# IntelLabs/GKL

Hardware: AMD Instinct MI355X
Metric: pairhmm_gcups (higher is better)
Workload: dtype f32

## Files before the change

gkl_amd/csrc/pairhmm_aux_kernels.h:

```cpp
#pragma once
#include <hip/hip_runtime.h>
#include <stdint.h>

#include "../../include/gkl_hip_pairhmm.h"
#include "pairhmm_fwd_kernel.h"
#include "pairhmm_multi_sets.h"

namespace gklhip {

struct PrepArgs {
  const uint8_t* hap_bases;
  const int32_t* hap_src;
  const int32_t* hap_len;
  const int32_t* hap_pos;
  const int32_t* hap_group;
  const int32_t* hap_pos_flat;
  uint32_t* stream_flat;
  uint32_t* stream;
  uint8_t* hap_has_n;
  int32_t n_haps;
  int32_t* clear_a; int32_t n_a;
  int32_t* clear_b; int32_t n_b;
  int32_t* clear_c; int32_t n_c;
  const uint4* pull_src; uint4* pull_dst; int32_t pull_n16;
// ... 166 lines not shown
  a.b.del = global_ptr(a.b.del); a.b.gcp = global_ptr(a.b.gcp); a.b.read_off = global_ptr(a.b.read_off);
  a.tab.ph2pr = global_ptr(a.tab.ph2pr); a.tab.div3 = global_ptr(a.tab.div3); a.tab.mm = global_ptr(a.tab.mm);
  a.stream = global_ptr(a.stream); a.hap_len = global_ptr(a.hap_len); a.hap_pos = global_ptr(a.hap_pos);
  a.hap_orig = global_ptr(a.hap_orig); a.y0 = global_ptr(a.y0); a.hap_has_n = global_ptr(a.hap_has_n);
  a.groups = global_ptr(a.groups); a.chunk_lanes = global_ptr(a.chunk_lanes); a.raw = global_ptr(a.raw);
  fwd_stream_block<double, kRplJobs, FMA>(a, block, lds);
}
__global__ __launch_bounds__(kFlagBlock) void finalize64_multi_kernel(MultiArgs m) {
  const int r = multi_find(m, (int)blockIdx.x);
  const SmallCall* c = m.call[r];
  const int p = multi_local(m.begin, r, (int)blockIdx.x) * kFlagBlock + (int)threadIdx.x;
  if (p >= c->n_pairs) return;
  c->q.used64[p] = 1;
  reinterpret_cast<uint64_t*>(c->q.out)[p] = packed_word(c->d.raw[p]);
}

constexpr int kModePacked = kModePackedWords;

struct FinalizeArgs {
  const float* raw32;
  const double* raw64;
  double* out;
  uint8_t* used64;
  int32_t* count;
  int32_t* read_fail;
  int32_t n_haps;
  int64_t n;
  int mode;
  float log10_init_f;
  double log10_init32_as_f64;
  double log10_init_d;
};

__global__ void finalize32_kernel(FinalizeArgs a) {
  const int64_t i = (int64_t)blockIdx.x * blockDim.x + threadIdx.x;
  if (i >= a.n || a.used64[i]) return;
  const float v = a.raw32[i];
  if (a.mode == GKLHIP_FINALIZE_DEVICE_F64) a.out[i] = log10((double)v) - a.log10_init32_as_f64;
  else if (a.mode == GKLHIP_FINALIZE_DEVICE_REF32) a.out[i] = (double)((float)log10((double)v) - a.log10_init_f);
}

__global__ void finalize64_kernel(FinalizeArgs a, int all_pairs) {
  const int64_t p = (int64_t)blockIdx.x * blockDim.x + threadIdx.x;
  if (p >= a.n) return;
  if (all_pairs) a.used64[p] = 1;
  else if (!a.used64[p]) return;
  if (a.mode >= 0) a.out[p] = log10(a.raw64[p]) - a.log10_init_d;
  if (a.mode == kModePacked) reinterpret_cast<uint64_t*>(a.out)[p] = packed_word(a.raw64[p]);
}

#ifndef GKL_PACK_WINDOW
#define GKL_PACK_WINDOW 96
#endif
constexpr int kPackWindow = GKL_PACK_WINDOW;
constexpr int kJobClasses = 64;
constexpr int kPlanBlock = 1024;

struct PlanArgs {
  FinalizeArgs fa;
  int32_t n_reads, n_haps, n_pairs_i;
  const int64_t* read_off;
  int32_t rpl;
  int32_t max_len;
  int32_t* cnts;
  int32_t* hist;
  int32_t* pos;
  int32_t* order;
  LaneSlot* lanes2;
  const int32_t* hap_orig;
  const int32_t* hap_group;
  const int32_t* hap_pos;
  const int32_t* hap_len;
  FwdJob* jobs;
  FwdJob* sorted;
  const LaneSlot* long_lanes;
  int32_t n_long;
  FwdJob* jobs_long;
  int32_t* long_chunk_jobs;
  int32_t total_cols;
  int32_t wanted_jobs;
  int32_t min_job_cols;
// ... 142 lines not shown
    for (int k = 0; k < kBatch; k++)
      if (f[k] > 0) a.order[atomicAdd(pos + f[k], 1)] = r0 + k * kPlanBlock;
  }
}

__global__ __launch_bounds__(kPlanBlock) void plan_policy_kernel(PlanArgs a) {
  __shared__ int32_t s_i32[kPlanBlock / 64];
  __shared__ int32_t s_wave[kPlanBlock / 64];
  __shared__ int32_t s_hist[2 * kPlanLdsBins];
  const int tid = (int)threadIdx.x, lane = tid & 63, wave = tid >> 6;
  const int nblk = (int)gridDim.x, blk = (int)blockIdx.x;

  {
    int32_t my_fails = 0;
    for (int64_t base = (int64_t)blk * kPlanBlock; base < a.fa.n; base += (int64_t)nblk * kPlanBlock) {
      const int64_t i = base + tid;
      const bool in_range = i < a.fa.n;
      const float v = in_range ? a.fa.raw32[i] : 1.0f;
      const bool fails = in_range && v < 1e-28f;
      const uint64_t mask = __ballot(fails);
      if (mask) {
        const int leader = __builtin_ctzll(mask);
        const int32_t read = fails ? (int32_t)((uint32_t)i / (uint32_t)a.n_haps) : -1;
        const int32_t lead_read = __shfl(read, leader, 64);
        const uint64_t same = __ballot(fails && read == lead_read);
        if (lane == leader) atomicAdd(a.fa.read_fail + lead_read, __builtin_popcountll(same));
        if (fails && read != lead_read) atomicAdd(a.fa.read_fail + read, 1);
        if (lane == 0) my_fails += __builtin_popcountll(mask);
      }
      if (in_range) {
        a.fa.used64[i] = fails ? 1 : 0;
        if (a.fa.mode == kModePacked && !a.packed_by_kernels)
          reinterpret_cast<uint64_t*>(a.fa.out)[i] = fails ? 0ull : (kPackedF32Tag | (uint64_t)__float_as_uint(v));
      }
    }
    if (lane == 0) s_wave[wave] = my_fails;
    __syncthreads();
    if (tid == 0) {
      int total = 0;
      for (int w = 0; w < kPlanBlock / 64; w++) total += s_wave[w];
      if (total) atomicAdd(a.cnts + 0, total);
    }
  }
  if (!last_block_done(a.cnts + 10)) return;
  const int n_fail = ld_cnt(a.cnts + 0);
  if (n_fail == 0) return;
  const uint64_t clk0 = wall_clock64();

  if (a.n_haps + 2 <= kPlanLdsBins) order_affected_reads<true>(a, s_hist, s_hist + kPlanLdsBins, s_i32, tid, clk0);
  else                             order_affected_reads<false>(a, a.hist, a.pos, s_i32, tid, clk0);
  GKLHIP_PLAN_STAMP(2);
}

__global__ __launch_bounds__(kPlanBlock) void plan_pack_kernel(PlanArgs a) {
  const int tid = (int)threadIdx.x, lane = tid & 63, wave = tid >> 6;
  const int nblk = (int)gridDim.x, blk = (int)blockIdx.x;
  if (ld_cnt(a.cnts + 0) == 0) return;
  const uint64_t clk0 = wall_clock64();

  {
    static_assert(kPackWindow <= 2 * kLanes, "the window's lane counts sit in two registers per lane");
    __shared__ int32_t s_pack[kPlanBlock / 64][4][kPackWindow];
    int32_t* s_read = s_pack[wave][0]; int32_t* s_needl = s_pack[wave][1]; int32_t* s_sread = s_pack[wave][2];
    int32_t* s_sneed = s_pack[wave][3];
    const int n = ld_cnt(a.cnts + 4);
    const int n_win = (n + kPackWindow - 1) / kPackWindow;
// ... 360 lines not shown
```

gkl_amd/csrc/pairhmm_ctx.h:

```cpp
#pragma once

using namespace gklhip;

namespace {
struct EnvSwitches {
  static bool on_unless_zero(const char* name) { const char* v = getenv(name); return !v || atoi(v) != 0; }
  static int integer(const char* name) { const char* v = getenv(name); return v ? atoi(v) : 0; }
  const bool wide_long = on_unless_zero("GKLHIP_WIDE_LONG");
  const bool super_long = on_unless_zero("GKLHIP_SUPER_LONG");
  const bool fused_pairs = on_unless_zero("GKLHIP_FUSED_PAIRS");
  const int64_t fused_max = [] { const char* v = getenv("GKLHIP_FUSED_MAX_PAIRS"); return v ? atoll(v) : -1LL; }();
  const bool xcd_aware = on_unless_zero("GKLHIP_XCD_AWARE");
  const bool timing = getenv("GKLHIP_TIMING") != nullptr;
  const int combine_load = integer("GKL_HIP_COMBINE_LOAD");
  const int target_cols = integer("GKLHIP_TARGET_COLS");
  const int fb_wanted_jobs = integer("GKLHIP_FB_WANTED_JOBS");
  const int plan_blocks = integer("GKLHIP_PLAN_BLOCKS");
  const int finalize_threads = integer("GKL_HIP_FINALIZE_THREADS");
  const int finalize_min = integer("GKL_HIP_FINALIZE_MIN");
  const bool combine = [] { const char* v = getenv("GKL_HIP_COMBINE"); return !(v && v[0] == '0'); }();
  const bool combine_mid = integer("GKL_HIP_COMBINE_MID") != 0;
  const bool quiet = getenv("GKL_HIP_QUIET") != nullptr;
  const bool one_device_engine = integer("GKL_HIP_DEVICE_ENGINES") == 1;
  const int small_read_limit = integer("GKL_HIP_SMALL_READ_LIMIT") == 511 ? 511 : 383;
// ... 3 lines not shown

#include "hip_host_common.h"

struct DevCtx {
  gklhip_config cfg;
  int device = 0;
  bool multi_device = false;
  int n_cus = 256;
  int n_xcds = 8;
  int asm_general = 1;
  int speculate_fp64 = 0;
  int small_read_limit = g_env.small_read_limit;
  int mid_combine = g_env.combine_mid ? 1 : 0;
  int lds_oob_zero = 1;
  hipStream_t stream = nullptr;
  DevBuf tab32, tab64;
  DevTables<float> dt32;
  DevTables<double> dt64;
  PinBuf stage_slot[2];
  DevBuf plan_dev_slot[2];
  hipEvent_t stage_free_slot[2] = {nullptr, nullptr};
  hipEvent_t plan_unused_slot[2] = {nullptr, nullptr};
  hipStream_t upload_stream = nullptr;
  bool upload_eager = false;
  hipStream_t pad_stream = nullptr;
  int plan_slot = 0;
  DevBuf raw32, raw64, used64, counters, stream_buf, out_dev;
  DevBuf lanes_main;
  DevBuf read_fail, lanes2, jobs, jobs_long, fail_order, fail_hist, hap_flags;
  DevBuf batch_dev;
  PinBuf res_pin;
  WorkerPool workers;
  hipStream_t copy_stream = nullptr;
  hipEvent_t policy_done = nullptr, early_copy_done = nullptr;
  hipEvent_t call_done = nullptr;
  bool have_call_done = false;
  static constexpr int kEventRing = 64;
  hipEvent_t ev_ring[kEventRing][6] = {};
  hipEvent_t* ev = ev_ring[0];
  int64_t calls = 0;
  bool ring_double[kEventRing] = {};
  gklhip_stats stats;
  int64_t last_pairs = 0;
  hipStream_t last_stream = nullptr;
  bool have_last = false;
  Plan plan;
  std::vector<PlanLane> long_lanes;
  std::vector<FwdJob> long_jobs;
  DevBuf carry;
};
```

gkl_amd/csrc/pairhmm_ctx_lifecycle.h:

```cpp
#pragma once

namespace {

std::atomic<int> g_eager_upload_holders{0};

int trim_streams(DevCtx* c) {
  if (!c->copy_stream && !c->pad_stream && (!c->upload_stream || c->upload_eager)) return 0;
  (void)hipSetDevice(c->device);
  for (hipStream_t s : {c->stream, c->copy_stream, c->upload_stream, c->have_last ? c->last_stream : nullptr})
    if (s && hipStreamQuery(s) != hipSuccess) { (void)hipGetLastError(); return 0; }
  int n = 0;
  if (c->copy_stream) { (void)hipStreamDestroy(c->copy_stream); c->copy_stream = nullptr; n++; }
  if (c->pad_stream) { (void)hipStreamDestroy(c->pad_stream); c->pad_stream = nullptr; n++; }
  if (c->upload_stream && !c->upload_eager) { (void)hipStreamDestroy(c->upload_stream); c->upload_stream = nullptr; n++; }
  return n;
}

void dev_done(DevCtx* c) {
  if (!c) return;
  (void)hipSetDevice(c->device);
  if (c->upload_eager) g_eager_upload_holders--;
  if (c->stream) (void)hipStreamSynchronize(c->stream);
  if (c->last_stream && c->have_last) (void)hipStreamSynchronize(c->last_stream);
  for (DevBuf* b : {&c->tab32, &c->tab64, &c->plan_dev_slot[0], &c->plan_dev_slot[1], &c->raw32, &c->raw64, &c->used64,
                    &c->counters, &c->stream_buf, &c->out_dev, &c->batch_dev, &c->read_fail, &c->lanes_main,
                    &c->lanes2, &c->jobs, &c->jobs_long, &c->fail_order, &c->fail_hist, &c->carry, &c->hap_flags})
    b->release();
  c->stage_slot[0].release();
  c->stage_slot[1].release();
  c->res_pin.release();
  if (c->policy_done) (void)hipEventDestroy(c->policy_done);
  if (c->early_copy_done) (void)hipEventDestroy(c->early_copy_done);
  if (c->call_done) (void)hipEventDestroy(c->call_done);
  if (c->copy_stream) { (void)hipStreamSynchronize(c->copy_stream); (void)hipStreamDestroy(c->copy_stream); }
  for (auto& set : c->ev_ring)
    for (auto& e : set) if (e) (void)hipEventDestroy(e);
  for (int k = 0; k < 2; k++) {
    if (c->stage_free_slot[k]) (void)hipEventDestroy(c->stage_free_slot[k]);
    if (c->plan_unused_slot[k]) (void)hipEventDestroy(c->plan_unused_slot[k]);
  }
  if (c->upload_stream) { (void)hipStreamSynchronize(c->upload_stream); (void)hipStreamDestroy(c->upload_stream); }
  if (c->pad_stream) (void)hipStreamDestroy(c->pad_stream);
  if (c->stream) (void)hipStreamDestroy(c->stream);
  delete c;
}

int dev_init(const gklhip_config& cfg, int dev, int ndev, DevCtx** out) {
  *out = nullptr;
  if (dev < 0 || dev >= ndev) return fail(GKLHIP_ERR_INVALID_ARG, "device %d of %d", dev, ndev);
  HIP_TRY(hipSetDevice(dev));
  {
    static const char* sched = getenv("GKL_HIP_SCHEDULE");
    if (sched && *sched) {
      const unsigned f = strcmp(sched, "yield") == 0 ? hipDeviceScheduleYield : strcmp(sched, "blocking") == 0 ? hipDeviceScheduleBlockingSync
                         : strcmp(sched, "spin") == 0 ? hipDeviceScheduleSpin : hipDeviceScheduleAuto;
      (void)hipSetDeviceFlags(f);
      (void)hipGetLastError();
    }
  }
  hipDeviceProp_t prop;
  HIP_TRY(hipGetDeviceProperties(&prop, dev));
  if (strncmp(prop.gcnArchName, "gfx950", 6) != 0)
    return fail(GKLHIP_ERR_NO_DEVICE, "device %d is %s; this library is built for gfx950 only", dev, prop.gcnArchName);
  DevCtx* c = new (std::nothrow) DevCtx();
  if (!c) return fail(GKLHIP_ERR_OOM, "context allocation failed");
  c->cfg = cfg;
// ... 35 lines not shown
      if (oob_checked[(size_t)dev] < 0)
        fprintf(stderr, "[gklhip] pairhmm: LDS reads beyond the allocation do not return 0 on device %d (%08x): the fp32 general steps stay in C++\n", dev, h_out[2]);
    }
    if (checked[(size_t)dev] < 0)
      return bail(fail(GKLHIP_ERR_HIP, "this library was built without the denormal-flush flags its kernels depend on (gkl_amd/csrc/Makefile: HIPFLAGS)"));
    c->lds_oob_zero = oob_checked[(size_t)dev] > 0 ? 1 : 0;
  }
  {
    const char* ag = getenv("GKLHIP_ASM_GENERAL");
    c->asm_general = ag ? (atoi(ag) != 0) : 1;
    const char* sp = getenv("GKLHIP_SPECULATE_FP64");
    c->speculate_fp64 = sp ? (atoi(sp) != 0) : 0;
    const char* sf = getenv("GKLHIP_SELFTEST_FAIL");
    if (sf && strcmp(sf, "lds_oob") == 0) {
      c->lds_oob_zero = 0;
      fprintf(stderr, "[gklhip] pairhmm: GKLHIP_SELFTEST_FAIL=lds_oob: the fp32 general steps stay in C++ for this context\n");
    }
  }
  if (g_eager_upload_holders.fetch_add(1) == 0) {
    if (hipStreamCreateWithFlags(&c->upload_stream, hipStreamNonBlocking) != hipSuccess) { g_eager_upload_holders--; return bail(fail(GKLHIP_ERR_HIP, "hipStreamCreate failed")); }
    c->upload_eager = true;
  } else {
    g_eager_upload_holders--;
  }
  if (const char* v = getenv("GKL_HIP_EAGER_STREAMS")) {
    const int k = atoi(v);
    if (k >= 7) { if (aux_streams(c) != GKLHIP_OK) return bail(GKLHIP_ERR_HIP); }
    else for (int i = 0; i < k; i++) { hipStream_t d = nullptr; (void)hipStreamCreateWithFlags(&d, hipStreamNonBlocking); }
  }
  for (int k = 0; k < 2; k++)
    if (hipEventCreateWithFlags(&c->stage_free_slot[k], hipEventDisableTiming) != hipSuccess ||
        hipEventCreateWithFlags(&c->plan_unused_slot[k], hipEventDisableTiming) != hipSuccess)
      return bail(fail(GKLHIP_ERR_HIP, "hipEventCreate failed"));
  if (hipEventCreateWithFlags(&c->policy_done, hipEventDisableTiming) != hipSuccess ||
      hipEventCreateWithFlags(&c->early_copy_done, hipEventDisableTiming) != hipSuccess ||
      hipEventCreateWithFlags(&c->call_done, hipEventDisableTiming) != hipSuccess)
    return bail(fail(GKLHIP_ERR_HIP, "hipEventCreate failed"));
  for (int k = 0; k < 2; k++)
    if (hipEventRecord(c->stage_free_slot[k], c->stream) != hipSuccess || hipEventRecord(c->plan_unused_slot[k], c->stream) != hipSuccess)
      return bail(fail(GKLHIP_ERR_HIP, "hipEventRecord failed"));
  {
    const int sets = c->cfg.record_events == 2 ? DevCtx::kEventRing : 1;
    for (int k = 0; k < sets; k++)
      for (auto& e : c->ev_ring[k])
        if (hipEventCreate(&e) != hipSuccess) return bail(fail(GKLHIP_ERR_HIP, "hipEventCreate failed"));
  }
  if ((rc = upload_tables(c, host_tables_f32(), &c->tab32, &c->dt32))) return bail(rc);
  if ((rc = upload_tables(c, host_tables_f64(), &c->tab64, &c->dt64))) return bail(rc);
  *out = c;
  return GKLHIP_OK;
}

int lane_init(DevCtx* parent, DevCtx** out) {
  *out = nullptr;
  HIP_TRY(hipSetDevice(parent->device));
  DevCtx* c = new (std::nothrow) DevCtx();
  if (!c) return fail(GKLHIP_ERR_OOM, "context allocation failed");
  c->cfg = parent->cfg;
  c->device = parent->device;
  c->n_cus = parent->n_cus;
  c->n_xcds = parent->n_xcds;
  c->asm_general = parent->asm_general;
  c->speculate_fp64 = parent->speculate_fp64;
  c->small_read_limit = parent->small_read_limit;
  c->mid_combine = parent->mid_combine;
  c->lds_oob_zero = parent->lds_oob_zero;
  c->dt32 = parent->dt32;
  c->dt64 = parent->dt64;
  memset(&c->stats, 0, sizeof c->stats);
// ... 14 lines not shown
```

gkl_amd/csrc/pairhmm_device_pass.h:

```cpp
#pragma once

namespace {

int aux_streams(DevCtx* c) {
  if (!c->upload_stream) HIP_TRY(hipStreamCreateWithFlags(&c->upload_stream, hipStreamNonBlocking));
  if (!c->copy_stream) {
    HIP_TRY(hipStreamCreateWithFlags(&c->copy_stream, hipStreamNonBlocking));
    if (!c->pad_stream) HIP_TRY(hipStreamCreateWithFlags(&c->pad_stream, hipStreamNonBlocking));
  }
  return GKLHIP_OK;
}

template <typename T>
int upload_tables(DevCtx* c, const HostTables<T>& h, DevBuf* buf, DevTables<T>* dt) {
  const size_t n = (size_t)kQuals * 2 + kMmEntries;
  int st = buf->reserve(n * sizeof(T));
  if (st) return st;
  T* base = buf->as<T>();
  {
    T* pin = nullptr;
    HIP_TRY(hipHostMalloc(reinterpret_cast<void**>(&pin), n * sizeof(T), hipHostMallocDefault));
    memcpy(pin, h.ph2pr.data(), kQuals * sizeof(T));
    memcpy(pin + kQuals, h.div3.data(), kQuals * sizeof(T));
    memcpy(pin + 2 * kQuals, h.mm.data(), kMmEntries * sizeof(T));
// ... 51 lines not shown
  l.desc = o; if (inline_read_bytes) o = align_up(o + sizeof(SmallCall));
  l.total = o;
  return l;
}

int validate(const gklhip_batch* b) {
  if (!b) return fail(GKLHIP_ERR_INVALID_ARG, "batch is NULL");
  if (b->n_reads < 0 || b->n_haps < 0) return fail(GKLHIP_ERR_INVALID_ARG, "negative batch size");
  if (b->n_reads == 0 || b->n_haps == 0) return GKLHIP_OK;
  if (!b->read_off || !b->hap_off) return fail(GKLHIP_ERR_INVALID_ARG, "offset arrays are NULL");
  if (!b->read_bases || !b->read_quals || !b->ins_gop || !b->del_gop || !b->gcp || !b->hap_bases)
    return fail(GKLHIP_ERR_INVALID_ARG, "a batch byte array is NULL");
  if (b->read_off[0] != 0 || b->hap_off[0] != 0)
    return fail(GKLHIP_ERR_INVALID_ARG, "offset arrays must start at 0");
  for (int r = 0; r < b->n_reads; r++)
    if (b->read_off[r + 1] <= b->read_off[r])
      return fail(GKLHIP_ERR_INVALID_ARG, "read %d is empty or offsets are not increasing", r);
  for (int h = 0; h < b->n_haps; h++)
    if (b->hap_off[h + 1] <= b->hap_off[h])
      return fail(GKLHIP_ERR_INVALID_ARG, "haplotype %d is empty or offsets are not increasing", h);
  if ((int64_t)b->n_reads * b->n_haps >= (int64_t)1 << 31)
    return fail(GKLHIP_ERR_UNSUPPORTED, "more than 2^31 pairs in one call");
  if (b->hap_off[b->n_haps] + b->n_haps + 4096 >= (int64_t)1 << 31)
    return fail(GKLHIP_ERR_UNSUPPORTED, "haplotype bases exceed 2^31");
  return GKLHIP_OK;
}

template <typename T, int RPL>
void launch_stream(const FwdArgs<T>& a, int fma, int n_blocks, hipStream_t s) {
  if (fma) hipLaunchKernelGGL((pairhmm_fwd_stream_kernel<T, RPL, true>), dim3(n_blocks), dim3(64), 0, s, a);
  else     hipLaunchKernelGGL((pairhmm_fwd_stream_kernel<T, RPL, false>), dim3(n_blocks), dim3(64), 0, s, a);
}
template <typename T, int RPL>
void launch_jobs(const FwdArgs<T>& a, int fma, int n_blocks, hipStream_t s) {
  if (fma) hipLaunchKernelGGL((pairhmm_fwd_jobs_kernel<T, RPL, true>), dim3(n_blocks), dim3(64), 0, s, a);
  else     hipLaunchKernelGGL((pairhmm_fwd_jobs_kernel<T, RPL, false>), dim3(n_blocks), dim3(64), 0, s, a);
}

template <typename T, int RPL>
void launch_long(const FwdArgs<T>& a, int fma, int n_blocks, T* carry, int carry_len, hipStream_t s) {
  if (fma) hipLaunchKernelGGL((pairhmm_fwd_long_kernel<T, RPL, true>), dim3(n_blocks), dim3(64), 0, s, a, carry, carry_len);
  else     hipLaunchKernelGGL((pairhmm_fwd_long_kernel<T, RPL, false>), dim3(n_blocks), dim3(64), 0, s, a, carry, carry_len);
}

template <typename T> constexpr int super_waves() { return 7; }
template <typename T> constexpr int super_blocks_max() { return sizeof(T) == 8 ? 256 : 512; }
inline int64_t super_steps(int carry_len, int max_read_len, int rpl) { return (int64_t)carry_len + 64 * (int64_t)((blocks_for(max_read_len, rpl) + kLanes - 1) / kLanes); }
template <typename T, int RPL, int RPL_STRIPED>
void launch_long_jobs(const FwdArgs<T>& a, int fma, int n_blocks, int max_read_len, T* carry, int carry_len, hipStream_t s,
                      unsigned char* xcarry = nullptr, int64_t xsteps = 0, int32_t* next2 = nullptr) {
  const bool wide_env = g_env.wide_long, super_env = g_env.super_long;
  if (!wide_env) { launch_long<T, RPL_STRIPED>(a, fma, n_blocks, carry, carry_len, s); return; }
  if (super_env && xcarry && next2 && (blocks_for(max_read_len, RPL) + kLanes - 1) / kLanes > kWideWavesMax) {
    static_assert(RPL == kRplSuper, "the super-stripe kernel's array depth");
    FwdArgs<T> sa = a;
    sa.super_steps = xsteps;
    if (fma) hipLaunchKernelGGL((pairhmm_fwd_super_kernel<T, RPL, super_waves<T>(), true>), dim3(std::min(n_blocks, super_blocks_max<T>())), dim3(64 * (super_waves<T>() + 1)), 0, s, sa, xcarry);
    else     hipLaunchKernelGGL((pairhmm_fwd_super_kernel<T, RPL, super_waves<T>(), false>), dim3(std::min(n_blocks, super_blocks_max<T>())), dim3(64 * (super_waves<T>() + 1)), 0, s, sa, xcarry);
    sa.long_filter = 2;
    sa.job_next = next2;
    launch_long<T, RPL_STRIPED>(sa, fma, n_blocks, carry, carry_len, s);
    return;
  }
  const int waves = std::max(2, std::min(kWideWavesMax, (blocks_for(max_read_len, RPL) + kLanes - 1) / kLanes));
  if (fma) {
    if (waves == 2)      hipLaunchKernelGGL((pairhmm_fwd_wide_kernel<T, RPL, true, 2>), dim3(n_blocks), dim3(128), 0, s, a, carry, carry_len);
    else if (waves == 3) hipLaunchKernelGGL((pairhmm_fwd_wide_kernel<T, RPL, true, 3>), dim3(n_blocks), dim3(192), 0, s, a, carry, carry_len);
    else                 hipLaunchKernelGGL((pairhmm_fwd_wide_kernel<T, RPL, true, 4>), dim3(n_blocks), dim3(256), 0, s, a, carry, carry_len);
  } else {
// ... 301 lines not shown
    copy_six_arrays(*db, L.batch_stride, [dst](size_t at, const uint8_t* src, size_t n) { memcpy(dst + at, src, n); return 0; });
    build_host_streams(hs, L, plan, db->hap_bases, n_haps);
  }
}

struct StagedCall {
  hipStream_t s;
  double* out;
  int slot;
  unsigned char* hs;
  const unsigned char* hs_dev;
  unsigned char* dp;
  DevBatch b;
  const uint8_t* hap_bases;
  uint32_t *stream_grouped, *stream_flat;
  uint8_t *hap_has_n, *xcarry;
};

int stage_call(DevCtx* c, const gklhip_batch* db, const CallPlan& P, double* out_dev, hipStream_t s, StagedCall* out) {
  const PlanLayout& L = P.L;
  const Plan& plan = c->plan;
  StagedCall& S = *out;
  int rc;
  const int slot = c->plan_slot ^= 1;
  PinBuf& stage = c->stage_slot[slot];
  DevBuf& plan_dev = c->plan_dev_slot[slot];
  HIP_TRY(hipEventSynchronize(c->stage_free_slot[slot]));
  if (L.total > stage.cap || L.total > plan_dev.cap) HIP_TRY(hipEventSynchronize(c->plan_unused_slot[slot]));
  if ((rc = stage.reserve(L.total))) return rc;
  if ((rc = plan_dev.reserve(L.total))) return rc;
  unsigned char* hs = stage.as<unsigned char>();
  fill_plan_block(hs, P, plan, c->long_lanes, c->long_jobs, db);
  unsigned char* dp = plan_dev.as<unsigned char>();
  if (c->have_call_done && c->last_stream != s) HIP_TRY(hipStreamWaitEvent(s, c->call_done, 0));
  S.hs_dev = nullptr;
  if (P.pull) {
    void* p = nullptr;
    HIP_TRY(hipHostGetDevicePointer(&p, hs, 0));
    S.hs_dev = static_cast<const unsigned char*>(p);
    if (!P.defers) HIP_TRY(hipStreamWaitEvent(s, c->plan_unused_slot[slot], 0));
  } else {
    if ((rc = aux_streams(c))) return rc;
    HIP_TRY(hipStreamWaitEvent(c->upload_stream, c->plan_unused_slot[slot], 0));
    HIP_TRY(hipMemcpyAsync(dp, hs, L.total, hipMemcpyHostToDevice, c->upload_stream));
    HIP_TRY(hipEventRecord(c->stage_free_slot[slot], c->upload_stream));
    HIP_TRY(hipStreamWaitEvent(s, c->stage_free_slot[slot], 0));
  }
  if (g_env.timing)
    fprintf(stderr, "[gklhip] host plan + staging: %.3f ms (%d chunks, %d stream entries, %zu plan bytes)\n",
            std::chrono::duration<double, std::milli>(std::chrono::steady_clock::now() - P.t0).count(),
            plan.n_chunks, plan.n_stream, L.total);

  if ((rc = c->raw32.reserve((size_t)P.n_pairs * 4))) return rc;
  if ((rc = c->raw64.reserve((size_t)P.n_pairs * 8))) return rc;
  if ((rc = c->used64.reserve((size_t)P.n_pairs))) return rc;
  if ((rc = c->counters.reserve(128))) return rc;
  if ((rc = c->read_fail.reserve((size_t)P.n_reads * 4))) return rc;
  if ((rc = c->stream_buf.reserve(((size_t)plan.n_stream + (size_t)plan.n_stream_flat) * 4))) return rc;
  if (!P.use_double && (rc = c->fail_hist.reserve((size_t)P.n_hist * 4))) return rc;
  if ((rc = c->hap_flags.reserve((size_t)P.n_haps))) return rc;
  if ((rc = c->lanes_main.reserve((size_t)std::max(plan.n_chunks, 1) * kLanes * sizeof(LaneSlot)))) return rc;

  S.s = s; S.out = out_dev; S.slot = slot; S.hs = hs; S.dp = dp; S.xcarry = nullptr;
  const gklhip_batch dbi = P.inline_host ? batch_at(*db, dp + L.batch, L.batch_stride) : *db;
  S.b = DevBatch{dbi.read_bases, dbi.read_quals, dbi.ins_gop, dbi.del_gop, dbi.gcp, reinterpret_cast<const int64_t*>(dp + L.read_off), P.n_reads, P.n_haps};
  S.hap_bases = (P.pull && P.inline_host) ? batch_at(*db, S.hs_dev + L.batch, L.batch_stride).hap_bases : dbi.hap_bases;
  S.stream_grouped = P.inline_host ? reinterpret_cast<uint32_t*>(dp + L.stream) : c->stream_buf.as<uint32_t>();
// ... 189 lines not shown
  if (P.fused) {
    if (int rc = launch_pair_fused(a, d, q, P.rows, P.fma, P.n_pairs, s, c->speculate_fp64 && g_host_calls_in_flight.load(std::memory_order_relaxed) <= 1)) return rc;
  } else if (P.n_pairs > kTwoStepFrom) {
    if (int rc = c->fail_order.reserve((size_t)P.n_pairs * 4)) return rc;
    if (int rc = launch_pair_policy_two_step(d, q, P.rows, P.fma, P.n_pairs, c->fail_order.as<int32_t>(), s)) return rc;
  } else {
    if (int rc = launch_pair_policy(d, q, P.rows, P.fma, P.n_pairs, s)) return rc;
  }
  if (ev) HIP_TRY(hipEventRecord(c->ev[4], s));
  HIP_TRY(hipEventRecord(c->policy_done, s));
  return GKLHIP_OK;
}
int launch_planned_fp64(DevCtx* c, const CallPlan& P, const StagedCall& S) {
  const bool ev = c->cfg.record_events != 0;
  hipStream_t s = S.s;
  const int n_reads = P.n_reads;
  const int64_t n_pairs = P.n_pairs;
  const size_t max_jobs = planned_max_jobs(P);
  int rc;
  if ((rc = c->fail_order.reserve(((size_t)n_reads + (size_t)P.n_long64) * 4))) return rc;
  if ((rc = c->lanes2.reserve((size_t)n_reads * kLanes * sizeof(LaneSlot)))) return rc;
  if ((rc = c->jobs.reserve(2 * max_jobs * sizeof(FwdJob)))) return rc;
  if (P.n_long64 > 0 && (rc = c->jobs_long.reserve((size_t)P.n_long64 * (size_t)P.n_haps * sizeof(FwdJob)))) return rc;
  const PlanArgs pa = plan_args(c, P, S);
  const int blocks_env = g_env.plan_blocks;
  const int policy_grid = std::max(1, blocks_env > 0 ? blocks_env : (int)std::min<int64_t>(c->n_cus, std::max<int64_t>(16, n_pairs / 4096)));
  const int64_t max_windows = ((int64_t)n_reads + kPackWindow - 1) / kPackWindow;
  const int pack_grid = (int)std::max<int64_t>(1, std::min<int64_t>(kPlanBlocks, (max_windows + kPlanBlock / 64 - 1) / (kPlanBlock / 64)));
  const int jobs_grid = std::max(1, std::min(c->n_cus, blocks_env > 0 ? blocks_env : (int)std::min<int64_t>(kPlanBlocks, std::max<int64_t>(16, n_pairs / 8192))));
  hipLaunchKernelGGL(plan_policy_kernel, dim3((unsigned)policy_grid), dim3(kPlanBlock), 0, s, pa);
  HIP_TRY(hipEventRecord(c->policy_done, s));
  hipLaunchKernelGGL(plan_pack_kernel, dim3((unsigned)pack_grid), dim3(kPlanBlock), 0, s, pa);
  hipLaunchKernelGGL(plan_jobs_kernel, dim3((unsigned)jobs_grid), dim3(kPlanBlock), 0, s, pa);
  const bool side_finalize = finalizes_on_device(P.finalize_mode);
  if (side_finalize) {
    if ((rc = aux_streams(c))) return rc;
    HIP_TRY(hipStreamWaitEvent(c->copy_stream, c->policy_done, 0));
    hipLaunchKernelGGL(finalize32_kernel, dim3((unsigned)((n_pairs + 255) / 256)), dim3(256), 0, c->copy_stream, pa.fa);
    HIP_TRY(hipEventRecord(c->early_copy_done, c->copy_stream));
  }
  FwdArgs<double> d = recompute_args(c, P, S);
  d.chunk_lanes = c->lanes2.as<LaneSlot>();
  d.n_chunks = n_reads;
  d.jobs = c->jobs.as<FwdJob>() + max_jobs;
  if (ev) HIP_TRY(hipEventRecord(c->ev[3], s));
  launch_jobs<double, kRplF64Jobs>(d, P.fma, (int)std::min<int64_t>(n_pairs, (int64_t)c->n_cus * 16), s);
  if (P.n_long64 > 0) {
    int32_t* cnts = c->counters.as<int32_t>();
    FwdArgs<double> ld = d;
    ld.chunk_lanes = pa.long_lanes;
    ld.jobs = c->jobs_long.as<FwdJob>();
    ld.job_count = cnts + 8;
    ld.job_next = cnts + 9;
    launch_long_jobs<double, kRplF64Wide, kRplF64>(ld, P.fma, P.n_long_waves, c->plan.max_read_len, c->carry.as<double>(), P.carry_len, s, S.xcarry, P.xsteps, cnts + 13);
  }
  if (ev) HIP_TRY(hipEventRecord(c->ev[4], s));
  hipLaunchKernelGGL(finalize64_kernel, dim3((unsigned)((n_pairs + 255) / 256)), dim3(256), 0, s, pa.fa, 0);
  if (side_finalize) HIP_TRY(hipStreamWaitEvent(s, c->early_copy_done, 0));
  return GKLHIP_OK;
}
int finish_call(DevCtx* c, const CallPlan& P, const StagedCall& S) {
  const bool ev = c->cfg.record_events != 0;
  hipStream_t s = S.s;
  gklhip_stats& st = c->stats;
  if (ev) HIP_TRY(hipEventRecord(c->ev[5], s));
  HIP_TRY(hipGetLastError());

  HIP_TRY(hipEventRecord(c->plan_unused_slot[S.slot], s));
  HIP_TRY(hipEventRecord(c->call_done, s));
  c->have_call_done = true;
  c->last_pairs = P.n_pairs;
  c->last_stream = s;
  c->have_last = true;

  if (ev && c->cfg.record_events != 2) {
    HIP_TRY(hipEventSynchronize(c->ev[5]));
    float ms = 0;
    HIP_TRY(hipEventElapsedTime(&ms, c->ev[1], c->ev[2])); st.ms_fwd_main = ms;
    HIP_TRY(hipEventElapsedTime(&ms, c->ev[3], c->ev[4])); st.ms_fwd_fallback = P.use_double ? 0.f : ms;
    HIP_TRY(hipEventElapsedTime(&ms, c->ev[0], c->ev[5])); st.ms_total_device = ms;
    int32_t cnt[2] = {0, 0};
    HIP_TRY(hipMemcpyAsync(cnt, c->counters.p, 8, hipMemcpyDeviceToHost, s));
    HIP_TRY(hipStreamSynchronize(s));
    st.n_fallback = P.use_double ? P.n_pairs : cnt[0];
    if (g_env.timing && !P.use_double) {
      int32_t k[32];
      HIP_TRY(hipMemcpy(k, c->counters.p, sizeof k, hipMemcpyDeviceToHost));
      fprintf(stderr, "[gklhip] policy+plan phases, each from the start of its own launch (us): hist %.1f scan %.1f scatter %.1f pack %.1f jobs %.1f sort %.1f | "
              "%d affected reads, %d chunks, %d jobs | window 0: loaded %.1f ranked %.1f fitted %.1f cleared %.1f written %.1f\n",
              k[16] * 0.01, k[17] * 0.01, k[18] * 0.01, k[19] * 0.01, k[20] * 0.01, k[21] * 0.01,
              k[4], k[5], k[2], k[22] * 0.01, k[23] * 0.01, k[24] * 0.01, k[25] * 0.01, k[26] * 0.01);
    }
  } else {
    st.n_fallback = P.use_double ? P.n_pairs : -1;
  }
  return GKLHIP_OK;
}

int32_t small_call_kind(const CallPlan& P) {
  if (P.use_double && P.n_pairs > kSmallDoublePairs) return kSmallDoubleStream;
  return P.pair_double ? kSmallDouble : P.fused ? kSmallFused : P.n_pairs > kTwoStepFrom ? kSmallTwoStep : kSmallOneLaunch;
}
// ... 53 lines not shown
```

gkl_amd/csrc/pairhmm_fwd_kernel.h:

```cpp
#pragma once
#include <hip/hip_runtime.h>
#include <stdint.h>

#include "pairhmm_pair_forms.h"

namespace gklhip {

constexpr uint32_t kEntIdle = 5u;
constexpr uint32_t kEntSep = 0x80000000u;
constexpr int kLanes = kPairLanes;
typedef const uint32_t __attribute__((address_space(4))) StreamWord;
}
#include "pairhmm_fwd_asm.h"
#ifndef GKLHIP_FAST_ASM
#define GKLHIP_FAST_ASM 1
#endif
namespace gklhip {

template <typename T>
struct DevTables {
  const T* ph2pr;
  const T* div3;
  const T* mm;
};
// ... 22 lines not shown
  int32_t klass;
};

template <typename T>
struct FwdArgs {
  DevBatch b;
  DevTables<T> tab;
  const uint32_t* stream;
  const int32_t* hap_len;
  const int32_t* hap_pos;
  const int32_t* hap_orig;
  const T* y0;
  const uint8_t* hap_has_n;
  const HapGroup* groups;
  int32_t n_groups;
  const LaneSlot* chunk_lanes;
  int32_t n_chunks;
  int32_t chunk_stride;
  T* raw;
  uint64_t* packed_out;
  const uint8_t* packed_only_flagged;
  const FwdJob* jobs;
  const int32_t* job_count;
  int32_t* job_next;
  int32_t asm_general;
  int32_t long_filter;
  int64_t super_steps;
};

constexpr uint64_t kPackedF32Tag = 0xFFFFFFFF00000000ull;
__device__ __forceinline__ uint64_t packed_word(double raw) {
  const uint64_t bits = (uint64_t)__double_as_longlong(raw);
  return (bits & kPackedF32Tag) == kPackedF32Tag ? 0x7FF8000000000000ull : bits;
}

template <typename T>
__device__ __forceinline__ void emit_result(const FwdArgs<T>& a, int64_t idx, T v) {
  a.raw[idx] = v;
  if (a.packed_out) {
    if (sizeof(T) == 4) {
      const float f = (float)v;
      a.packed_out[idx] = f < 1e-28f ? 0ull : (kPackedF32Tag | (uint64_t)__float_as_uint(f));
    } else if (!a.packed_only_flagged || a.packed_only_flagged[idx]) {
      a.packed_out[idx] = packed_word((double)v);
    }
  }
}

__device__ __forceinline__ uint32_t dpp_shr1_keep(uint32_t old, uint32_t src) {
  return (uint32_t)__builtin_amdgcn_update_dpp((int)old, (int)src, 0x138, 0xf, 0xf, false);
}
__device__ __forceinline__ uint32_t dpp_shr1_zero(uint32_t src) {
  return (uint32_t)__builtin_amdgcn_update_dpp(0, (int)src, 0x138, 0xf, 0xf, true);
}
__device__ __forceinline__ uint32_t dpp_shr1_and_nop(uint32_t src, uint32_t mask) {
  uint32_t d;
  asm("s_nop 1\n\tv_and_b32_dpp %0, %1, %2 wave_shr:1 row_mask:0xf bank_mask:0xf bound_ctrl:1" : "=v"(d) : "v"(src), "v"(mask));
  return d;
}
__device__ __forceinline__ float recv_above(float v, uint32_t lmask) {
  return __uint_as_float(dpp_shr1_and_nop(__float_as_uint(v), lmask));
}
__device__ __forceinline__ double recv_above(double v, uint32_t lmask) {
  const uint64_t u = (uint64_t)__double_as_longlong(v);
  const uint32_t lo = dpp_shr1_zero((uint32_t)u) & lmask;
  const uint32_t hi = dpp_shr1_zero((uint32_t)(u >> 32)) & lmask;
// ... 434 lines not shown
          const T bM = read_lane(M[RPL - 1], kLanes - 1), bX = read_lane(X[RPL - 1], kLanes - 1),
                  bY = read_lane(Y[RPL - 1], kLanes - 1);
          if (lane == (p & 63)) { coM = bM; coX = bX; coY = bY; }
          if ((p & 63) == 63 || t == t_end - 1) {
            const int base = p & ~63;
            cout[base + lane] = coM; cout[clen + base + lane] = coX; cout[2 * clen + base + lane] = coY;
          }
        }
      }
    }
  }
};

template <typename T, int RPL, bool FMA>
__device__ __forceinline__ void fwd_stream_block(const FwdArgs<T>& a, int block, unsigned char* lds) {
  using Job = WaveJob<T, RPL, FMA>;
  const int lane = threadIdx.x;
  const int g = block / a.chunk_stride;
  const int chunk = block - g * a.chunk_stride;
  if (chunk >= a.n_chunks) return;
  const HapGroup grp = a.groups[g];
  Job job;
  job.lds = lds;
  job.setup(a, lane, a.chunk_lanes[(int64_t)chunk * kLanes + lane]);
  __syncthreads();
  job.run(a, lane, grp.hap_begin, grp.hap_end);
}
template <typename T, int RPL, bool FMA>
__global__ __launch_bounds__(64) __attribute__((amdgpu_waves_per_eu(sizeof(T) == 8 ? 2 : 4))) void pairhmm_fwd_stream_kernel(FwdArgs<T> a) {
  __shared__ __attribute__((aligned(16))) unsigned char lds[WaveJob<T, RPL, FMA>::kLdsBytes];
  fwd_stream_block<T, RPL, FMA>(a, (int)blockIdx.x, lds);
}

template <typename T, int RPL, bool FMA>
__global__ __launch_bounds__(64) __attribute__((amdgpu_waves_per_eu(sizeof(T) == 8 ? 2 : 4))) void pairhmm_fwd_jobs_kernel(FwdArgs<T> a) {
  using Job = WaveJob<T, RPL, FMA>;
  __shared__ __attribute__((aligned(16))) unsigned char lds[Job::kLdsBytes];
  const int lane = threadIdx.x;
  const int n = *a.job_count;
  Job job;
  job.lds = lds;
  int loaded_chunk = INT32_MIN;
  for (;;) {
    int idx = 0;
    if (lane == 0) idx = atomicAdd(a.job_next, 1);
    idx = __builtin_amdgcn_readfirstlane(idx);
    if (idx >= n) break;
    const FwdJob j = a.jobs[idx];
    if (j.chunk != loaded_chunk) {
      __syncthreads();
      job.setup(a, lane, a.chunk_lanes[(int64_t)j.chunk * kLanes + lane]);
      __syncthreads();
      loaded_chunk = j.chunk;
    }
    job.run(a, lane, j.hap_begin, j.hap_end);
  }
}

struct PairPolicyArgs {
  const float* raw32;
  double* out;
  uint8_t* used64;
  int32_t* count;
  const int32_t* hap_sidx;
  int32_t mode;
  float log10_init_f;
  double log10_init32_as_f64, log10_init_d;
};
constexpr int kModePackedWords = -2;

__device__ __forceinline__ void pair_store_fp32(const PairPolicyArgs& q, int64_t p, float v) {
  if (q.mode == kModePackedWords) reinterpret_cast<uint64_t*>(q.out)[p] = kPackedF32Tag | (uint64_t)__float_as_uint(v);
  else if (q.mode == 1) q.out[p] = log10((double)v) - q.log10_init32_as_f64;
  else if (q.mode == 2) q.out[p] = (double)((float)log10((double)v) - q.log10_init_f);
}
__device__ __forceinline__ bool pair_policy_head(const PairPolicyArgs& q, int64_t p, int lane) {
  const float v = q.raw32[p];
  const bool fails = v < 1e-28f;
  if (lane == 0) q.used64[p] = fails ? 1 : 0;
  if (!fails) {
    if (lane == 0) pair_store_fp32(q, p, v);
    return false;
  }
  if (lane == 0) atomicAdd(q.count, 1);
  return true;
}
template <int RPL, bool FMA, bool MARK = false>
__device__ __forceinline__ void pair_policy_recompute(const FwdArgs<double>& a, const PairPolicyArgs& q, int64_t p, int r, int R, int k,
                                                      unsigned char* lds) {
  using Job = WaveJob<double, RPL, FMA>;
  const int lane = threadIdx.x & 63;
  LaneSlot slot;
  slot.read = lane < (R + RPL) / RPL ? r : -1;
  slot.block = lane;
  Job job;
  job.lds = lds;
  job.setup(a, lane, slot);
  __builtin_amdgcn_wave_barrier();
  job.run(a, lane, k, k + 1);
  if (job.out_read >= 0) {
    const double sum = a.raw[p];
    if (q.mode == kModePackedWords) reinterpret_cast<uint64_t*>(q.out)[p] = packed_word(sum);
// ... 449 lines not shown
```

gkl_amd/csrc/pairhmm_host_call.h:

```cpp
#pragma once

namespace {

struct HostCallInFlight {
  int share;
  HostCallInFlight() : share(g_host_calls_in_flight.fetch_add(1) + 1) {}
  ~HostCallInFlight() { g_host_calls_in_flight.fetch_sub(1); }
};
int finalize_threads(const DevCtx* c, int share) {
  const int env = g_env.finalize_threads;
  if (env > 0) return env;
  const int hw = (int)std::max(1u, std::thread::hardware_concurrency());
  int threads = c->cfg.max_threads;
  if (threads <= 0) threads = std::max(1, std::min(hw, 8) / std::max(1, share));
  return std::max(1, std::min(threads, 64));
}

constexpr int kFlightSlots = 4;
struct SmallCombiner {
  struct Ticket {
    const SmallLaunch* sl = nullptr;
    int state = 0;
    hipEvent_t ev = nullptr;
    int rc = GKLHIP_OK;
// ... 216 lines not shown
    }
    l.unlock();
    if (t.state == 2) { g_err = t.err; return t.rc; }
    if (t.state == 1) HIP_TRY(hipEventSynchronize(t.ev));
    return GKLHIP_OK;
  }
};
SmallCombiner* small_combiner(int device) {
  static std::mutex mu;
  static std::vector<SmallCombiner*> all;
  std::lock_guard<std::mutex> l(mu);
  if ((int)all.size() <= device) all.resize((size_t)device + 1, nullptr);
  if (!all[(size_t)device]) {
    SmallCombiner* k = all[(size_t)device] = new SmallCombiner();
    k->device = device;
    if (const char* v = getenv("GKL_HIP_EAGER_STREAMS")) if (atoi(v) >= 7) k->make_streams();
    if (const char* v = getenv("GKL_HIP_COMBINE_FLIGHTS")) all[(size_t)device]->max_flights = std::max(1, std::min(kFlightSlots, atoi(v)));
    if (const char* v = getenv("GKL_HIP_COMBINE_MIN")) all[(size_t)device]->min_batch = std::max(0, std::min(kCombineMax, atoi(v)));
    if (const char* v = getenv("GKL_HIP_COMBINE_WAIT_US")) all[(size_t)device]->batch_wait_ns = (int64_t)std::max(0, atoi(v)) * 1000;
  }
  return all[(size_t)device];
}
int64_t one_pass_min() { return g_env.finalize_min > 0 ? g_env.finalize_min : 8192; }
int dev_compute_host_impl(DevCtx* c, const gklhip_batch* hb, double* out_host) {
  const int64_t n_pairs = (int64_t)hb->n_reads * hb->n_haps;
  HIP_TRY(hipSetDevice(c->device));
  hipStream_t s = c->stream;
  int rc;
  const bool inline_inputs = inputs_inline(hb);
  gklhip_batch db = *hb;
  if (!inline_inputs) {
    if ((rc = c->batch_dev.reserve(six_arrays_bytes(hb)))) return rc;
    unsigned char* d = c->batch_dev.as<unsigned char>();
    if (c->have_call_done && c->last_stream != s) HIP_TRY(hipStreamWaitEvent(s, c->call_done, 0));
    const size_t stride = align_up((size_t)hb->read_off[hb->n_reads]);
    if ((rc = copy_six_arrays(*hb, stride, [d, s](size_t at, const uint8_t* src, size_t n) -> int { HIP_TRY(hipMemcpyAsync(d + at, src, n, hipMemcpyHostToDevice, s)); return GKLHIP_OK; }))) return rc;
    db = batch_at(*hb, d, stride);
  }
  const int mode = c->cfg.finalize;
  if ((rc = c->res_pin.reserve((size_t)n_pairs * 8))) return rc;
  double* pin_out = nullptr;
  {
    void* p = nullptr;
    HIP_TRY(hipHostGetDevicePointer(&p, c->res_pin.p, 0));
    pin_out = static_cast<double*>(p);
  }
  if (finalizes_on_device(mode)) {
    if ((rc = run_device(c, &db, pin_out, mode, s, inline_inputs))) return rc;
    HIP_TRY(hipStreamSynchronize(s));
    memcpy(out_host, c->res_pin.p, (size_t)n_pairs * 8);
    return GKLHIP_OK;
  }
  const HostCallInFlight in_flight;
  const int threads = finalize_threads(c, in_flight.share);
  HostFinalizer fin;
  const bool may_defer = deferral_offered(inline_inputs) && (!c->have_call_done || hipEventQuery(c->call_done) == hipSuccess);
  (void)hipGetLastError();
  const int64_t t_call = SmallCombiner::now_ns();
  CallPlan P;
  plan_call(c, &db, kModePacked, inline_inputs, may_defer, call_load(may_defer), &P);
  const bool mid = !P.defers && may_defer && mid_call_combines(c, P);
  if (mid) P.defers = true;
  if (P.defers) {
    StagedCall S;
    SmallLaunch small;
    if ((rc = stage_call(c, &db, P, pin_out, s, &S))) return rc;
    if (mid && !P.use_double && (rc = c->fail_order.reserve((size_t)P.n_pairs * 4))) return rc;
    describe_small_call(c, P, S, &small);
    SmallCombiner* k = small_combiner(c->device);
    const int64_t t_staged = SmallCombiner::now_ns();
    if ((rc = k->run(small, s))) return rc;
    const int64_t t_done = SmallCombiner::now_ns();
    c->stats.n_fallback = fin.all(&c->workers, c->res_pin.as<uint64_t>(), out_host, n_pairs, threads, one_pass_min());
    k->ns_stage.fetch_add(t_staged - t_call, std::memory_order_relaxed);
    k->ns_run.fetch_add(t_done - t_staged, std::memory_order_relaxed);
    k->ns_finalize.fetch_add(SmallCombiner::now_ns() - t_done, std::memory_order_relaxed);
    return GKLHIP_OK;
  }
  if ((rc = launch_call(c, &db, P, pin_out, s))) return rc;
  if (c->cfg.use_double || n_pairs <= kOnePassPairs) {
    HIP_TRY(hipStreamSynchronize(s));
    c->stats.n_fallback = fin.all(&c->workers, c->res_pin.as<uint64_t>(), out_host, n_pairs, threads, one_pass_min());
    return GKLHIP_OK;
  }
  HIP_TRY(hipEventSynchronize(c->policy_done));
  fin.early(&c->workers, c->res_pin.as<uint64_t>(), out_host, n_pairs, threads);
  HIP_TRY(hipStreamSynchronize(s));
  c->stats.n_fallback = fin.late(&c->workers, c->res_pin.as<uint64_t>(), out_host, threads);
  return GKLHIP_OK;
// ... 160 lines not shown
```

Measured before the change: 4734.

## Fuse fp64 and fp32 finalization into jobs and plan kernels, drop side stream

Moves the fp32 device finalization into the plan kernel that already reads raw32 values. The fp64 finalization for recomputed pairs now happens inside the fp64 jobs kernel after each job, so the separate finalize64 launch runs only when long fp64 jobs exist. It also removes the side-stream finalize32 launch with its event and reuses the plan slot event as the call-done marker. This saves kernel launches and cross-stream synchronization, at the cost of extra work and an s_waitcnt plus atomic loads inside the jobs kernel.

```diff
diff --git a/gkl_amd/csrc/pairhmm_aux_kernels.h b/gkl_amd/csrc/pairhmm_aux_kernels.h
--- a/gkl_amd/csrc/pairhmm_aux_kernels.h
+++ b/gkl_amd/csrc/pairhmm_aux_kernels.h
@@ -222,10 +222,7 @@
   double log10_init_d;
 };
 
-__global__ void finalize32_kernel(FinalizeArgs a) {
-  const int64_t i = (int64_t)blockIdx.x * blockDim.x + threadIdx.x;
-  if (i >= a.n || a.used64[i]) return;
-  const float v = a.raw32[i];
+__device__ __forceinline__ void finalize32_store(const FinalizeArgs& a, int64_t i, float v) {
   if (a.mode == GKLHIP_FINALIZE_DEVICE_F64) a.out[i] = log10((double)v) - a.log10_init32_as_f64;
   else if (a.mode == GKLHIP_FINALIZE_DEVICE_REF32) a.out[i] = (double)((float)log10((double)v) - a.log10_init_f);
 }
@@ -235,8 +232,7 @@
   if (p >= a.n) return;
   if (all_pairs) a.used64[p] = 1;
   else if (!a.used64[p]) return;
-  if (a.mode >= 0) a.out[p] = log10(a.raw64[p]) - a.log10_init_d;
-  if (a.mode == kModePacked) reinterpret_cast<uint64_t*>(a.out)[p] = packed_word(a.raw64[p]);
+  finalize64_store(a.out, a.mode, a.log10_init_d, p, a.raw64[p]);
 }
 
 #ifndef GKL_PACK_WINDOW
@@ -445,6 +441,7 @@
         a.fa.used64[i] = fails ? 1 : 0;
         if (a.fa.mode == kModePacked && !a.packed_by_kernels)
           reinterpret_cast<uint64_t*>(a.fa.out)[i] = fails ? 0ull : (kPackedF32Tag | (uint64_t)__float_as_uint(v));
+        if (!fails) finalize32_store(a.fa, i, v);
       }
     }
     if (lane == 0) s_wave[wave] = my_fails;
diff --git a/gkl_amd/csrc/pairhmm_ctx.h b/gkl_amd/csrc/pairhmm_ctx.h
--- a/gkl_amd/csrc/pairhmm_ctx.h
+++ b/gkl_amd/csrc/pairhmm_ctx.h
@@ -59,9 +59,10 @@
   PinBuf res_pin;
   WorkerPool workers;
   hipStream_t copy_stream = nullptr;
-  hipEvent_t policy_done = nullptr, early_copy_done = nullptr;
-  hipEvent_t call_done = nullptr;
+  hipEvent_t policy_done = nullptr;
+  int call_done_slot = 0;
   bool have_call_done = false;
+  hipEvent_t call_done() const { return plan_unused_slot[call_done_slot]; }
   static constexpr int kEventRing = 64;
   hipEvent_t ev_ring[kEventRing][6] = {};
   hipEvent_t* ev = ev_ring[0];
diff --git a/gkl_amd/csrc/pairhmm_ctx_lifecycle.h b/gkl_amd/csrc/pairhmm_ctx_lifecycle.h
--- a/gkl_amd/csrc/pairhmm_ctx_lifecycle.h
+++ b/gkl_amd/csrc/pairhmm_ctx_lifecycle.h
@@ -30,8 +30,6 @@
   c->stage_slot[1].release();
   c->res_pin.release();
   if (c->policy_done) (void)hipEventDestroy(c->policy_done);
-  if (c->early_copy_done) (void)hipEventDestroy(c->early_copy_done);
-  if (c->call_done) (void)hipEventDestroy(c->call_done);
   if (c->copy_stream) { (void)hipStreamSynchronize(c->copy_stream); (void)hipStreamDestroy(c->copy_stream); }
   for (auto& set : c->ev_ring)
     for (auto& e : set) if (e) (void)hipEventDestroy(e);
@@ -133,9 +131,7 @@
     if (hipEventCreateWithFlags(&c->stage_free_slot[k], hipEventDisableTiming) != hipSuccess ||
         hipEventCreateWithFlags(&c->plan_unused_slot[k], hipEventDisableTiming) != hipSuccess)
       return bail(fail(GKLHIP_ERR_HIP, "hipEventCreate failed"));
-  if (hipEventCreateWithFlags(&c->policy_done, hipEventDisableTiming) != hipSuccess ||
-      hipEventCreateWithFlags(&c->early_copy_done, hipEventDisableTiming) != hipSuccess ||
-      hipEventCreateWithFlags(&c->call_done, hipEventDisableTiming) != hipSuccess)
+  if (hipEventCreateWithFlags(&c->policy_done, hipEventDisableTiming) != hipSuccess)
     return bail(fail(GKLHIP_ERR_HIP, "hipEventCreate failed"));
   for (int k = 0; k < 2; k++)
     if (hipEventRecord(c->stage_free_slot[k], c->stream) != hipSuccess || hipEventRecord(c->plan_unused_slot[k], c->stream) != hipSuccess)
diff --git a/gkl_amd/csrc/pairhmm_device_pass.h b/gkl_amd/csrc/pairhmm_device_pass.h
--- a/gkl_amd/csrc/pairhmm_device_pass.h
+++ b/gkl_amd/csrc/pairhmm_device_pass.h
@@ -107,9 +107,9 @@
   else     hipLaunchKernelGGL((pairhmm_fwd_stream_kernel<T, RPL, false>), dim3(n_blocks), dim3(64), 0, s, a);
 }
 template <typename T, int RPL>
-void launch_jobs(const FwdArgs<T>& a, int fma, int n_blocks, hipStream_t s) {
-  if (fma) hipLaunchKernelGGL((pairhmm_fwd_jobs_kernel<T, RPL, true>), dim3(n_blocks), dim3(64), 0, s, a);
-  else     hipLaunchKernelGGL((pairhmm_fwd_jobs_kernel<T, RPL, false>), dim3(n_blocks), dim3(64), 0, s, a);
+void launch_jobs(const FwdArgs<T>& a, const JobFinalize& f, int fma, int n_blocks, hipStream_t s) {
+  if (fma) hipLaunchKernelGGL((pairhmm_fwd_jobs_kernel<T, RPL, true>), dim3(n_blocks), dim3(64), 0, s, a, f);
+  else     hipLaunchKernelGGL((pairhmm_fwd_jobs_kernel<T, RPL, false>), dim3(n_blocks), dim3(64), 0, s, a, f);
 }
 
 template <typename T, int RPL>
@@ -477,7 +477,7 @@
   unsigned char* hs = stage.as<unsigned char>();
   fill_plan_block(hs, P, plan, c->long_lanes, c->long_jobs, db);
   unsigned char* dp = plan_dev.as<unsigned char>();
-  if (c->have_call_done && c->last_stream != s) HIP_TRY(hipStreamWaitEvent(s, c->call_done, 0));
+  if (c->have_call_done && c->last_stream != s) HIP_TRY(hipStreamWaitEvent(s, c->call_done(), 0));
   S.hs_dev = nullptr;
   if (P.pull) {
     void* p = nullptr;
@@ -733,19 +733,14 @@
   HIP_TRY(hipEventRecord(c->policy_done, s));
   hipLaunchKernelGGL(plan_pack_kernel, dim3((unsigned)pack_grid), dim3(kPlanBlock), 0, s, pa);
   hipLaunchKernelGGL(plan_jobs_kernel, dim3((unsigned)jobs_grid), dim3(kPlanBlock), 0, s, pa);
-  const bool side_finalize = finalizes_on_device(P.finalize_mode);
-  if (side_finalize) {
-    if ((rc = aux_streams(c))) return rc;
-    HIP_TRY(hipStreamWaitEvent(c->copy_stream, c->policy_done, 0));
-    hipLaunchKernelGGL(finalize32_kernel, dim3((unsigned)((n_pairs + 255) / 256)), dim3(256), 0, c->copy_stream, pa.fa);
-    HIP_TRY(hipEventRecord(c->early_copy_done, c->copy_stream));
-  }
   FwdArgs<double> d = recompute_args(c, P, S);
   d.chunk_lanes = c->lanes2.as<LaneSlot>();
   d.n_chunks = n_reads;
   d.jobs = c->jobs.as<FwdJob>() + max_jobs;
+  const bool jobs_finalize = P.n_long64 == 0;
+  const JobFinalize jf{pa.fa.out, pa.fa.log10_init_d, jobs_finalize ? pa.fa.mode : -1};
   if (ev) HIP_TRY(hipEventRecord(c->ev[3], s));
-  launch_jobs<double, kRplF64Jobs>(d, P.fma, (int)std::min<int64_t>(n_pairs, (int64_t)c->n_cus * 16), s);
+  launch_jobs<double, kRplF64Jobs>(d, jf, P.fma, (int)std::min<int64_t>(n_pairs, (int64_t)c->n_cus * 16), s);
   if (P.n_long64 > 0) {
     int32_t* cnts = c->counters.as<int32_t>();
     FwdArgs<double> ld = d;
@@ -756,8 +751,7 @@
     launch_long_jobs<double, kRplF64Wide, kRplF64>(ld, P.fma, P.n_long_waves, c->plan.max_read_len, c->carry.as<double>(), P.carry_len, s, S.xcarry, P.xsteps, cnts + 13);
   }
   if (ev) HIP_TRY(hipEventRecord(c->ev[4], s));
-  hipLaunchKernelGGL(finalize64_kernel, dim3((unsigned)((n_pairs + 255) / 256)), dim3(256), 0, s, pa.fa, 0);
-  if (side_finalize) HIP_TRY(hipStreamWaitEvent(s, c->early_copy_done, 0));
+  if (!jobs_finalize) hipLaunchKernelGGL(finalize64_kernel, dim3((unsigned)((n_pairs + 255) / 256)), dim3(256), 0, s, pa.fa, 0);
   return GKLHIP_OK;
 }
 int finish_call(DevCtx* c, const CallPlan& P, const StagedCall& S) {
@@ -768,7 +762,7 @@
   HIP_TRY(hipGetLastError());
 
   HIP_TRY(hipEventRecord(c->plan_unused_slot[S.slot], s));
-  HIP_TRY(hipEventRecord(c->call_done, s));
+  c->call_done_slot = S.slot;
   c->have_call_done = true;
   c->last_pairs = P.n_pairs;
   c->last_stream = s;
diff --git a/gkl_amd/csrc/pairhmm_fwd_kernel.h b/gkl_amd/csrc/pairhmm_fwd_kernel.h
--- a/gkl_amd/csrc/pairhmm_fwd_kernel.h
+++ b/gkl_amd/csrc/pairhmm_fwd_kernel.h
@@ -78,6 +78,11 @@
 __device__ __forceinline__ uint64_t packed_word(double raw) {
   const uint64_t bits = (uint64_t)__double_as_longlong(raw);
   return (bits & kPackedF32Tag) == kPackedF32Tag ? 0x7FF8000000000000ull : bits;
+}
+constexpr int kModePackedWords = -2;
+__device__ __forceinline__ void finalize64_store(double* out, int mode, double log10_init_d, int64_t p, double raw) {
+  if (mode >= 0) out[p] = log10(raw) - log10_init_d;
+  if (mode == kModePackedWords) reinterpret_cast<uint64_t*>(out)[p] = packed_word(raw);
 }
 
 template <typename T>
@@ -578,8 +583,34 @@
   fwd_stream_block<T, RPL, FMA>(a, (int)blockIdx.x, lds);
 }
 
+struct JobFinalize {
+  double* out;
+  double log10_init_d;
+  int32_t mode;
+};
+template <typename T>
+__device__ __forceinline__ void finalize_job_pairs(const FwdArgs<T>& a, const JobFinalize& f, int out_read, int hap_begin, int hap_end, int lane) {
+  static_assert(sizeof(T) == 8, "the packed fp64 recomputation pass");
+  asm volatile("s_waitcnt vmcnt(0)" ::: "memory");
+  const bool names = out_read >= 0;
+  const uint64_t m = __ballot(names);
+  const int n_r = __builtin_popcountll(m), below = __builtin_popcountll(m & ((1ull << lane) - 1ull));
+  const int reads = __builtin_amdgcn_ds_permute((names ? below : n_r + lane - below) << 2, out_read);
+  const int nh = hap_end - hap_begin, total = n_r * nh;
+  for (int i0 = 0; i0 < total; i0 += kLanes) {
+    const int i = i0 + lane;
+    const bool in = i < total;
+    const int ri = in ? (int)((uint32_t)i / (uint32_t)nh) : 0;
+    const int read = __builtin_amdgcn_ds_bpermute(ri << 2, reads);
+    if (in) {
+      const int64_t p = (int64_t)read * a.b.n_haps + a.hap_orig[hap_begin + (i - ri * nh)];
+      const double raw = __longlong_as_double(__hip_atomic_load(reinterpret_cast<const long long*>(a.raw + p), __ATOMIC_RELAXED, __HIP_MEMORY_SCOPE_AGENT));
+      if (a.packed_only_flagged[p]) finalize64_store(f.out, f.mode, f.log10_init_d, p, raw);
+    }
+  }
+}
 template <typename T, int RPL, bool FMA>
-__global__ __launch_bounds__(64) __attribute__((amdgpu_waves_per_eu(sizeof(T) == 8 ? 2 : 4))) void pairhmm_fwd_jobs_kernel(FwdArgs<T> a) {
+__global__ __launch_bounds__(64) __attribute__((amdgpu_waves_per_eu(sizeof(T) == 8 ? 2 : 4))) void pairhmm_fwd_jobs_kernel(FwdArgs<T> a, JobFinalize f) {
   using Job = WaveJob<T, RPL, FMA>;
   __shared__ __attribute__((aligned(16))) unsigned char lds[Job::kLdsBytes];
   const int lane = threadIdx.x;
@@ -600,6 +631,9 @@
       loaded_chunk = j.chunk;
     }
     job.run(a, lane, j.hap_begin, j.hap_end);
+    if constexpr (sizeof(T) == 8) {
+      if (f.mode != -1) finalize_job_pairs(a, f, job.out_read, j.hap_begin, j.hap_end, lane);
+    }
   }
 }
 
@@ -613,7 +647,6 @@
   float log10_init_f;
   double log10_init32_as_f64, log10_init_d;
 };
-constexpr int kModePackedWords = -2;
 
 __device__ __forceinline__ void pair_store_fp32(const PairPolicyArgs& q, int64_t p, float v) {
   if (q.mode == kModePackedWords) reinterpret_cast<uint64_t*>(q.out)[p] = kPackedF32Tag | (uint64_t)__float_as_uint(v);
diff --git a/gkl_amd/csrc/pairhmm_host_call.h b/gkl_amd/csrc/pairhmm_host_call.h
--- a/gkl_amd/csrc/pairhmm_host_call.h
+++ b/gkl_amd/csrc/pairhmm_host_call.h
@@ -272,7 +272,7 @@
   if (!inline_inputs) {
     if ((rc = c->batch_dev.reserve(six_arrays_bytes(hb)))) return rc;
     unsigned char* d = c->batch_dev.as<unsigned char>();
-    if (c->have_call_done && c->last_stream != s) HIP_TRY(hipStreamWaitEvent(s, c->call_done, 0));
+    if (c->have_call_done && c->last_stream != s) HIP_TRY(hipStreamWaitEvent(s, c->call_done(), 0));
     const size_t stride = align_up((size_t)hb->read_off[hb->n_reads]);
     if ((rc = copy_six_arrays(*hb, stride, [d, s](size_t at, const uint8_t* src, size_t n) -> int { HIP_TRY(hipMemcpyAsync(d + at, src, n, hipMemcpyHostToDevice, s)); return GKLHIP_OK; }))) return rc;
     db = batch_at(*hb, d, stride);
@@ -294,7 +294,7 @@
   const HostCallInFlight in_flight;
   const int threads = finalize_threads(c, in_flight.share);
   HostFinalizer fin;
-  const bool may_defer = deferral_offered(inline_inputs) && (!c->have_call_done || hipEventQuery(c->call_done) == hipSuccess);
+  const bool may_defer = deferral_offered(inline_inputs) && (!c->have_call_done || hipEventQuery(c->call_done()) == hipSuccess);
   (void)hipGetLastError();
   const int64_t t_call = SmallCombiner::now_ns();
   CallPlan P;
```

New measurement: 4742 (median of 4 runs). Within noise of the previous version (+0.2%).
